# ffs97/deep-mixture-vae

Measured on AMD Instinct MI355X. Metric: images/sec (train), MNIST K=10 z=64 batch=4096/GPU bf16, higher is better.
Workload: dtype bf16; 1 GPU; configs[1]: DMVAE MLP 784-500-500-(2000|2000)-z64/K10-2000-500-500-784, one ELBO training step (gather+fwd+loss+bwd+Adam), synthetic rows resident in HBM; per_gpu_batch=4096, global_batch=4096, parallelism=dp1, rccl_ranks=0, multi_rank_rccl_verified_before_this_run=False, hip_graph=True, float_atomics=False, update=adam fused into the dW launch, mode=exact (expectation over q(c|x), priors.py:130-145)

## Files before the change

### deep-mixture-vae_amd/build.py

```python
import os
import subprocess
import sys
from concurrent.futures import ThreadPoolExecutor

HERE = os.path.dirname(os.path.abspath(__file__))
CSRC = os.path.join(HERE, "csrc")
OUT = os.path.join(HERE, "dmvae_hip", "libdmvae_hip.so")
SOURCES = ["gemm_bf16.hip", "gemm_bf16_256.hip", "gemm_f32.hip", "latent.hip", "latent_mfma.hip", "latent_vade.hip", "latent_vade_mfma.hip", "elementwise.hip", "conv.hip", "heads_dx.hip", "heads_latent.hip", "strip_fwd2.hip", "moe_head.hip", "gmm_fit.hip", "gmm_seed.hip", "eval_clusters.hip", "api.hip"]
FLAGS = ["--offload-arch=gfx950", "-O3", "-fPIC", "-std=c++17", "-Wall", "-Wno-unused-function",
         "-mllvm", "-amdgpu-mfma-vgpr-form=1"]


def _stale(target, deps):
    if not os.path.exists(target):
        return True
    t = os.path.getmtime(target)
    return any(os.path.getmtime(d) > t for d in deps)


def build(force=False, verbose=True):
    hipcc = os.environ.get("HIPCC", "/opt/rocm/bin/hipcc")
    headers = [os.path.join(CSRC, f) for f in os.listdir(CSRC) if f.endswith(".h")]
    headers += [os.path.join(HERE, "..", "include", h) for h in ("dmvae_hip.h", "dmvae_hip_debug.h")]
    objdir = os.path.join(HERE, "build")
    os.makedirs(objdir, exist_ok=True)
    os.makedirs(os.path.dirname(OUT), exist_ok=True)
    jobs = []
    objs = []
    for src in SOURCES:
        sp = os.path.join(CSRC, src)
        op = os.path.join(objdir, src.replace(".hip", ".o"))
        objs.append(op)
        if force or _stale(op, [sp] + headers):
            jobs.append([hipcc] + FLAGS + ["-c", sp, "-o", op])

    def run(cmd):
        if verbose:
            print(" ".join(cmd), flush=True)
        r = subprocess.run(cmd, capture_output=True, text=True)
        if r.returncode != 0:
            raise RuntimeError("hipcc failed:\n%s\n%s" % (" ".join(cmd), r.stderr[-6000:]))
        if verbose and r.stderr.strip():
            print(r.stderr[-3000:], file=sys.stderr)

    with ThreadPoolExecutor(max_workers=min(4, max(1, len(jobs)))) as ex:
        list(ex.map(run, jobs))
    if jobs or force or _stale(OUT, objs):
        run([hipcc, "--offload-arch=gfx950", "-shared", "-fPIC", "-o", OUT] + objs)
    return OUT


def build_host_asan(verbose=False):
    import glob
    hipcc = os.environ.get("HIPCC", "/opt/rocm/bin/hipcc")
    objdir = os.path.join(HERE, "build", "asan")
    os.makedirs(objdir, exist_ok=True)
    out = os.path.join(objdir, "libdmvae_hip_asan.so")
    headers = [os.path.join(CSRC, f) for f in os.listdir(CSRC) if f.endswith(".h")] + [os.path.join(HERE, "..", "include", h) for h in ("dmvae_hip.h", "dmvae_hip_debug.h")]
    flags = ["--offload-arch=gfx950", "--cuda-host-only", "-O1", "-g", "-fPIC", "-std=c++17", "-fsanitize=address,undefined", "-fno-gpu-sanitize",
             "-fno-omit-frame-pointer", "-fno-sanitize-recover=undefined"]
    objs, jobs = [], []
    for src in SOURCES:
        sp, op = os.path.join(CSRC, src), os.path.join(objdir, src.replace(".hip", ".o"))
        objs.append(op)
        if _stale(op, [sp] + headers):
            jobs.append([hipcc] + flags + ["-c", sp, "-o", op])

    def run(cmd):
        if verbose:
            print(" ".join(cmd), flush=True)
        r = subprocess.run(cmd, capture_output=True, text=True)
        if r.returncode != 0:
            raise RuntimeError("hipcc (host asan) failed:\n%s\n%s" % (" ".join(cmd), r.stderr[-6000:]))
    with ThreadPoolExecutor(max_workers=min(4, max(1, len(jobs)))) as ex:
        list(ex.map(run, jobs))
    if jobs or _stale(out, objs):
        und = subprocess.run(["nm", "-u"] + objs, capture_output=True, text=True).stdout
        syms = sorted({w for line in und.splitlines() for w in line.split() if w.startswith("__hip_fatbin_")})
        stub = os.path.join(objdir, "fatbin_stubs.c")
        with open(stub, "w") as f:
            for sname in syms:
                f.write('const char %s[32] __attribute__((aligned(4096))) = "__CLANG_OFFLOAD_BUNDLE__";\n' % sname)
        run(["gcc", "-c", "-fPIC", stub, "-o", stub.replace(".c", ".o")])
        run([hipcc, "--offload-arch=gfx950", "--cuda-host-only", "-shared", "-fPIC", "-fsanitize=address,undefined", "-fno-gpu-sanitize", "-shared-libsan", "-o", out]
            + objs + [stub.replace(".c", ".o")])
    rt = sorted(glob.glob("/opt/rocm/lib/llvm/lib/clang/*/lib/linux/libclang_rt.asan-x86_64.so"))
    return out, (rt[-1] if rt else None)


if __name__ == "__main__":
    print(build(force="-f" in sys.argv))
```

### deep-mixture-vae_amd/csrc/api.hip

```cpp
#include <stdarg.h>
#include <stdlib.h>
#include <string.h>

#include <map>
#include <mutex>
#include <string>
#include <vector>

#include "kernels.h"
#include "moe_head.h"
#include "gmm_fit.h"
#include "gmm_seed.h"
#include "eval_clusters.h"
#include "measure.h"

namespace dmvae {

static thread_local char g_err[512] = "";
void set_error(const char* fmt, ...) {
    va_list ap;
    va_start(ap, fmt);
    vsnprintf(g_err, sizeof(g_err), fmt, ap);
    va_end(ap);
}
// ... 1376 lines not shown
    DMVAE_REQUIRE(out && n > 0, "dmvae_philox_uniform: bad argument");
    return philox_launch((hipStream_t)stream, out, n, seed, step, sid, 2);
}
extern "C" int dmvae_philox_gumbel(void* stream, float* out, int64_t n, uint64_t seed, uint64_t step, uint32_t sid) {
    DMVAE_REQUIRE(out && n > 0, "dmvae_philox_gumbel: bad argument");
    return philox_launch((hipStream_t)stream, out, n, seed, step, sid, 1);
}
extern "C" int dmvae_cast_f32_to_bf16(void* stream, const float* in, void* out, int64_t n) {
    DMVAE_REQUIRE(in && out && n > 0, "dmvae_cast: bad argument");
    return cast_launch((hipStream_t)stream, in, out, n, 1);
}
extern "C" int dmvae_cast_bf16_to_f32(void* stream, const void* in, float* out, int64_t n) {
    DMVAE_REQUIRE(in && out && n > 0, "dmvae_cast: bad argument");
    return cast_launch((hipStream_t)stream, in, out, n, 0);
}

extern "C" int dmvae_debug_spin(void* stream, int microseconds) { return spin_launch((hipStream_t)stream, microseconds); }
extern "C" int dmvae_debug_strip_fwd2(void* stream, int B_pad, int K0, const void* X, int64_t ldx, const void* W0, int64_t ld0, const float* b0,
                                      const void* W1, int64_t ld1, const float* b1, void* Y1, int64_t ldy1, void* Y2, int64_t ldy2) {
    return strip_fwd2_launch((hipStream_t)stream, B_pad, K0, X, ldx, W0, ld0, b0, W1, ld1, b1, Y1, ldy1, Y2, ldy2);
}
extern "C" int dmvae_debug_stamps(void** device_ptr) {
    if (!device_ptr) return DMVAE_EINVAL;
    *device_ptr = gemm_bf16_stamps();
    if (!*device_ptr) *device_ptr = heads_dx_phase_table();
    return *device_ptr ? 0 : DMVAE_ESTATE;
}

extern "C" int dmvae_debug_anatomy(void** device_ptr) {
    if (!device_ptr) return DMVAE_EINVAL;
    *device_ptr = gemm_bf16_anatomy();
    return *device_ptr ? 0 : DMVAE_ESTATE;
}
extern "C" int dmvae_debug_anatomy256(void** device_ptr) {
    if (!device_ptr) return DMVAE_EINVAL;
    *device_ptr = gemm_bf16_256_anatomy();
    return *device_ptr ? 0 : DMVAE_ESTATE;
}

extern "C" int dmvae_debug_conv_first_fwd(void* stream, int dtype, const void* x, int64_t bstride, int H, int64_t n_img, const void* W, int ldw,
                                          const float* bias, void* out, int ld) {
    DMVAE_REQUIRE((dtype == DMVAE_F32 || dtype == DMVAE_BF16) && x && W && bias && out && H > 0 && n_img > 0 && bstride >= (int64_t)H * H, "dmvae_debug_conv_first_fwd: bad argument");
    return conv_first_fwd_launch((hipStream_t)stream, dtype, x, bstride, H, n_img, W, ldw, bias, 32, out, ld);
}
extern "C" int dmvae_debug_conv_first_dw(void* stream, int dtype, const void* x, int64_t bstride, int H, int64_t n_img, const void* dY, int ld,
                                         float* dW, int ldw, float* db, float* part, int64_t part_floats, int* n_blocks) {
    DMVAE_REQUIRE((dtype == DMVAE_F32 || dtype == DMVAE_BF16) && H > 0 && H % 4 == 0 && n_img > 0 && (ld == 32 || ld == 64) && n_blocks &&
                  n_img * H * (H / 4) < (1ll << 31), "dmvae_debug_conv_first_dw: bad argument (side a multiple of 4, ld 32 or 64)");
    *n_blocks = conv_first_dw_blocks(H, n_img);
    if (!part) return 0;
    DMVAE_REQUIRE(x && dY && dW && db && bstride >= (int64_t)H * H && part_floats >= (int64_t)*n_blocks * 320,
                  "dmvae_debug_conv_first_dw: bad argument (scratch: %d blocks x 320 floats)", *n_blocks);
    return conv_first_dw_launch((hipStream_t)stream, dtype, x, bstride, H, n_img, dY, ld, 32, dW, ldw, db, part);
}
extern "C" int dmvae_debug_zero_border(void* stream, int dtype, void* a, int P, int ld, int64_t n_img) {
    DMVAE_REQUIRE((dtype == DMVAE_F32 || dtype == DMVAE_BF16) && a && P >= 2 && n_img > 0, "dmvae_debug_zero_border: bad argument");
    return zero_border_launch((hipStream_t)stream, dtype, a, P, ld, n_img);
}
extern "C" int dmvae_debug_maxpool2_fwd(void* stream, int dtype, const void* in, int H, int ld, int64_t n_img, void* out, int out_border) {
    DMVAE_REQUIRE((dtype == DMVAE_F32 || dtype == DMVAE_BF16) && in && out && H > 0 && n_img > 0 && (out_border == 0 || out_border == 1), "dmvae_debug_maxpool2_fwd: bad argument");
    return maxpool2_fwd_launch((hipStream_t)stream, dtype, in, H, ld, n_img, out, out_border);
}
extern "C" int dmvae_debug_maxpool2_bwd_relu(void* stream, int dtype, const void* in, const void* dout, int H, int ld, int64_t n_img, void* din, int dout_border) {
    DMVAE_REQUIRE((dtype == DMVAE_F32 || dtype == DMVAE_BF16) && in && dout && din && H > 0 && n_img > 0 && (dout_border == 0 || dout_border == 1), "dmvae_debug_maxpool2_bwd_relu: bad argument");
    return maxpool2_bwd_relu_launch((hipStream_t)stream, dtype, in, dout, H, ld, n_img, din, dout_border);
}
extern "C" int dmvae_debug_conv_wflip(void* stream, int dtype, const void* W, int cin, int cin_ld, int cout, int ldw, void* Wt, int Kt) {
    DMVAE_REQUIRE((dtype == DMVAE_F32 || dtype == DMVAE_BF16) && W && Wt && cin > 0 && cout > 0 && ldw >= cout, "dmvae_debug_conv_wflip: bad argument");
    return conv_wflip_launch((hipStream_t)stream, dtype, W, cin, cin_ld, cout, ldw, Wt, Kt);
}
extern "C" int dmvae_debug_conv_gemm(void* stream, int dtype, int layout, int M, int N, int K, const void* A, int64_t lda,
                                     const void* B, int64_t ldb, const dmvae_epilogue* epi, int split_k, int conv_p, int conv_c) {
    DMVAE_REQUIRE(conv_p >= 3 && conv_c > 0, "dmvae_debug_conv_gemm: conv_p = side + 2 >= 3, conv_c > 0");
    return gemm_checked((hipStream_t)stream, dtype, layout, M, N, K, A, lda, B, ldb, epi, split_k, nullptr, conv_p, conv_c);
}
extern "C" int dmvae_debug_conv_dw(void* stream, int dtype, int rows, int conv_p, int conv_c, const void* X, int64_t ldx, const void* dY, int64_t ldy,
                                   int N, int n_valid, int split, float* slab, float* dW, float* db) {
    DMVAE_REQUIRE(rows > 0 && conv_p >= 3 && conv_c > 0 && N > 0 && n_valid > 0 && n_valid <= N && dW && db && split >= 1 && rows % (split * 64) == 0 && (split == 1 || slab),
                  "dmvae_debug_conv_dw: bad argument");
    const int kdim = pad64(9 * conv_c);
    hipError_t me = hipMemsetAsync(dW, 0, (size_t)kdim * N * 4, (hipStream_t)stream);
    if (me == hipSuccess) me = hipMemsetAsync(db, 0, (size_t)N * 4, (hipStream_t)stream);
    if (me != hipSuccess) { set_error("dmvae_debug_conv_dw memset: %s", hipGetErrorString(me)); return (int)me; }
    return conv_layer_dw((hipStream_t)stream, dtype, rows, conv_p, conv_c, kdim, X, ldx, dY, ldy, N, n_valid, split, slab, dW, db);
}

extern "C" int dmvae_prof_enable(int on) {
    std::lock_guard<std::mutex> lk(g_prof_mu);
    g_prof_on = on != 0;
    return 0;
}
extern "C" int dmvae_prof_collect(dmvae_prof_row* rows, int max_rows) {
    std::lock_guard<std::mutex> lk(g_prof_mu);
    std::map<std::string, dmvae_prof_row> agg;
    std::vector<std::string> order;
    for (auto& r : g_prof) {
        (void)hipEventSynchronize(r.e1);
        float ms = 0.f;
        (void)hipEventElapsedTime(&ms, r.e0, r.e1);
        double kms = 0.0;
        bool kok = !r.k.empty();
        for (auto& pr : r.k) {
            float d = 0.f;
            if (hipEventSynchronize(pr.second) != hipSuccess || hipEventElapsedTime(&d, pr.first, pr.second) != hipSuccess || !(d > 0.f)) kok = false;
            kms += d;
            g_event_pool.push_back(pr.first);
            g_event_pool.push_back(pr.second);
        }
        (void)hipGetLastError();
        auto it = agg.find(r.name);
        if (it == agg.end()) {
            dmvae_prof_row row;
            memset(&row, 0, sizeof(row));
            snprintf(row.name, sizeof(row.name), "%s", r.name);
            it = agg.emplace(r.name, row).first;
            order.push_back(r.name);
        }
        it->second.launches += 1;
        it->second.total_ms += ms;
        it->second.kernel_ms += kok ? kms : 0.0;
        it->second.kernel_launches += kok ? (int64_t)r.k.size() : 0;
        it->second.flops += r.flops;
        it->second.bytes += r.bytes;
        g_event_pool.push_back(r.e0);
        g_event_pool.push_back(r.e1);
    }
    g_prof.clear();
    g_prof_cur = -1;
    int n = 0;
    for (auto& k : order) {
        if (n >= max_rows) break;
        rows[n++] = agg[k];
    }
    return n;
}

extern "C" int dmvae_debug_set_tile(int bm, int bn) {
    DMVAE_REQUIRE((bm == 0 && bn == 0) || ((bm == 64 || bm == 128) && (bn == 64 || bn == 128)), "dmvae_debug_set_tile: 64 or 128 (0,0 = heuristic)");
    gemm_bf16_force_tile(bm * 1000 + bn);
    return 0;
}

extern "C" int dmvae_debug_set_knob(int which, int value) {
    if (which == 10) { g_dw_slices = value; return 0; }
    if (which == 11) { g_dw_macro = value; return 0; }
    if (which == 12) { g_heads_dx_form = value; return 0; }
    if (which == 13) { heads_dx_stream_set(value); return 0; }
    if (which == 16) { g_fin_rides = value; return 0; }
    if (which == 17) { g_pf_rides = value; return 0; }
    if (which == 18 || which == 20) { gemm_bf16_set_knob(which, value); return 0; }
    if (which == 19) { heads_latent_set(value); return 0; }
    if (which == 21) { g_ksplit = value; return 0; }
    if (which == 22) { latent_vade_force_mfma(value); return 0; }
    if (which == 14) { latent_set_blocks_target(value); return 0; }
    DMVAE_REQUIRE(which >= 0 && which <= 9 && which != 3, "dmvae_debug_set_knob: knob 0 = supertile rows, 1 = 8-wave workgroups, 2 = per-problem tiles in grouped grids, (3: removed, the deep-ring policy), 4 = XCD runs per tile class in grouped grids, 5 = short-K conv tiles, 6 = 256x256 tile policy, 7 = short-K workgroups, 8 = first-tile stagger of the merged dW grid, 9 = waves per workgroup of a grouped dX launch; 10 / 11 = K slices of the dW groups, 12 = heads dX as one or two launches, 13 = heads dX on the streaming kernel (1) or the grouped tiles (0), 14 = blocks the latent kernel's geometry aims at (512), 19 = fused heads + latent launch, 20 = XCD partition of the grouped dW launch, 21 = K slices of a small batch's thin launches, 22 = VaDE's large-table latent form wherever the caller brings its scratch");
    gemm_bf16_set_knob(which, value);
    return 0;
}

extern "C" int dmvae_abi_version(void) { return DMVAE_ABI_VERSION; }
extern "C" const char* dmvae_last_error(void) { return g_err; }
```

### deep-mixture-vae_amd/csrc/gemm_bf16.hip

```cpp
#include <algorithm>
#include <cmath>
#include <functional>
#include <map>
#include <mutex>
#include <string>
#include <vector>

#include "gemm_tile.h"
#include "measure.h"

MEAS_TABLES_BF16

namespace dmvae {

template <int BM, int BN, int LAYOUT, int EPI, int NSTAGE, int NW, int BKT = BK, bool CONV = false, bool BONLY = false>
__device__ __forceinline__ void gemm_bf16_body(const GemmArgs& a, const int bid_raw, const int gstart, const int nwg, bf16_t* smem,
                                               const dmvae_adam_ctx* ac = nullptr, const int kslice = -1) {
    constexpr bool A_KC = (LAYOUT != DMVAE_GEMM_DW);
    constexpr bool B_KC = (LAYOUT == DMVAE_GEMM_DX);
    constexpr int A_ELEMS = BM * BKT, B_ELEMS = BN * BKT, STAGE = A_ELEMS + B_ELEMS;
    constexpr int WM = NW / 2;
    constexpr int TM = BM / (16 * WM), TN = BN / 32;
    static_assert(!BONLY || (LAYOUT == DMVAE_GEMM_DW && EPI == DMVAE_EPI_STORE_F32 && !CONV), "bias-only strips: dense DW / STORE_F32");
    constexpr int LOADS = ((BONLY ? 0 : BM) + BN) * BKT / (512 * NW);
// ... 756 lines not shown
    return check_launch("gemm_bf16_grouped");
}

int gemm_bf16_grouped(hipStream_t s, int layout, const GemmArgs* probs, int nprob, const dmvae_finalize_args* fin) {
    if (nprob < 1 || nprob > DMVAE_MAX_GROUP) { set_error("dmvae_gemm_grouped: 1..%d problems", DMVAE_MAX_GROUP); return DMVAE_EINVAL; }
    const int epi = probs[0].epi.kind;
    for (int i = 1; i < nprob; ++i)
        if (probs[i].epi.kind != epi) { set_error("dmvae_gemm_grouped: all problems must share the epilogue kind"); return DMVAE_EINVAL; }
    if (layout == DMVAE_GEMM_DW && epi == DMVAE_EPI_STORE_F32) return grouped_launch<DMVAE_GEMM_DW, DMVAE_EPI_STORE_F32>(s, probs, nprob);
    if (layout == DMVAE_GEMM_FWD && epi == DMVAE_EPI_BIAS_F32) return grouped_launch<DMVAE_GEMM_FWD, DMVAE_EPI_BIAS_F32>(s, probs, nprob);
    if (fin && !(layout == DMVAE_GEMM_DX && epi == DMVAE_EPI_RELU_MASK)) { set_error("dmvae_gemm_grouped: step_finalize rides on DX / RELU_MASK groups only"); return DMVAE_EINVAL; }
    if (layout == DMVAE_GEMM_DX && epi == DMVAE_EPI_RELU_MASK) {
        bool taken[DMVAE_MAX_GROUP];
        const int rc = heads_dx_stream_launch(s, probs, nprob, fin, taken);
        if (rc) return rc;
        GemmArgs rest[DMVAE_MAX_GROUP];
        int nrest = 0, ntaken = 0;
        for (int i = 0; i < nprob; ++i) {
            if (taken[i]) ++ntaken;
            else rest[nrest++] = probs[i];
        }
        if (nrest == 0) return 0;
        return grouped_launch<DMVAE_GEMM_DX, DMVAE_EPI_RELU_MASK>(s, rest, nrest, nullptr, ntaken ? nullptr : fin);
    }
    set_error("dmvae_gemm_grouped: layout %d with epilogue %d is not instantiated", layout, epi);
    return DMVAE_EUNSUPPORTED;
}
static int peel_large_dw(hipStream_t s, const GemmArgs* probs, int nprob, const dmvae_adam_ctx* ctx, std::vector<GemmArgs>& rest) {
    std::vector<GemmArgs> large;
    bool any = false;
    for (int i = 0; i < nprob; ++i)
        any = any || (probs[i].k_split == probs[i].K && gemm_bf16_256_ok(DMVAE_GEMM_DW, probs[i].epi.kind, probs[i].M, probs[i].N, probs[i].K, probs[i].conv_c != 0));
    for (int i = 0; i < nprob; ++i) {
        const GemmArgs& p = probs[i];
        if (p.k_split != p.K && !p.bias_only && !p.epi.out2 && p.slab_stride && gemm_bf16_256_slice_ok(p.M, p.N, p.k_split)) { large.push_back(p); continue; }
        const bool own = p.k_split == p.K && gemm_bf16_256_ok(DMVAE_GEMM_DW, p.epi.kind, p.M, p.N, p.K, p.conv_c != 0);
        const bool rides = any && gemm_bf16_256_rides() && p.k_split == p.K && !p.conv_c && p.M % 256 == 0 && p.N % 256 == 0 && p.K >= 1024 &&
                           (p.epi.kind == DMVAE_EPI_STORE_F32 || p.epi.kind == DMVAE_EPI_ADAM);
        if (own || rides) large.push_back(p);
        else rest.push_back(p);
    }
    return large.empty() ? 0 : gemm_bf16_256_dw_all(s, large.data(), (int)large.size(), ctx);
}
int gemm_bf16_grouped_dw(hipStream_t s, const GemmArgs* probs, int nprob) {
    if (nprob < 1 || nprob > DMVAE_MAX_GROUP) { set_error("dmvae_gemm_grouped_dw: 1..%d problems", DMVAE_MAX_GROUP); return DMVAE_EINVAL; }
    std::vector<GemmArgs> rest;
    for (int i = 0; i < nprob; ++i)
        if (probs[i].epi.kind != DMVAE_EPI_STORE_F32) return gemm_bf16_grouped(s, DMVAE_GEMM_DW, probs, nprob, nullptr);
    const int rc = peel_large_dw(s, probs, nprob, nullptr, rest);
    if (rc) return rc;
    return rest.empty() ? 0 : gemm_bf16_grouped(s, DMVAE_GEMM_DW, rest.data(), (int)rest.size(), nullptr);
}
int gemm_bf16_grouped_dw_adam(hipStream_t s, const GemmArgs* probs, int nprob, const dmvae_adam_ctx& ctx) {
    if (nprob < 1 || nprob > DMVAE_MAX_GROUP) { set_error("dmvae_gemm_grouped_dw_adam: 1..%d problems", DMVAE_MAX_GROUP); return DMVAE_EINVAL; }
    for (int i = 0; i < nprob; ++i)
        if (probs[i].epi.kind != DMVAE_EPI_ADAM || !probs[i].epi.out) { set_error("dmvae_gemm_grouped_dw_adam: every problem needs epilogue kind ADAM and out = its gradient address"); return DMVAE_EINVAL; }
    if (!ctx.param || !ctx.grad || !ctx.m || !ctx.v || !ctx.state || (ctx.seg_off & 3) || (ctx.seg_n & 3) || ctx.seg_n < 0) {
        set_error("dmvae_gemm_grouped_dw_adam: null arena / state, or a segment that is not a multiple of 4 elements");
        return DMVAE_EINVAL;
    }
    for (int i = 0; i < nprob; ++i) {
        const int64_t end = (reinterpret_cast<const float*>(probs[i].epi.out) - ctx.grad) + (int64_t)probs[i].M * probs[i].epi.ldo;
        if (end < 0 || end > ADAM_QUADS_MAX_ELEMS) { set_error("dmvae_gemm_grouped_dw_adam: gradient %d ends %lld elements into the arena (limit 2^30)", i, (long long)end); return DMVAE_EUNSUPPORTED; }
    }
    std::vector<GemmArgs> rest;
    dmvae_adam_ctx c1 = ctx;
    c1.seg_n = 0;
    const int rc = peel_large_dw(s, probs, nprob, &c1, rest);
    if (rc) return rc;
    if (!rest.empty()) return grouped_launch<DMVAE_GEMM_DW, DMVAE_EPI_ADAM>(s, rest.data(), (int)rest.size(), &ctx);
    if (ctx.seg_n > 0) {
        AdamArgs a;
        a.n = ctx.seg_n; a.p = ctx.param + ctx.seg_off; a.g = ctx.grad + ctx.seg_off; a.m = ctx.m + ctx.seg_off; a.v = ctx.v + ctx.seg_off;
        a.pb = ctx.param_bf16 ? reinterpret_cast<bf16_t*>(ctx.param_bf16) + ctx.seg_off : nullptr;
        a.lr = 0.f; a.b1 = ctx.beta1; a.b2 = ctx.beta2; a.eps = ctx.epsilon; a.gscale = ctx.grad_scale; a.zero_grad = 0; a.ieee = ctx.ieee;
        a.t_host = ~0ull; a.st = reinterpret_cast<const dmvae_state*>(ctx.state);
        return adam_launch(s, a);
    }
    return 0;
}

static int g_force_tile = 0;
void gemm_bf16_force_tile(int t) { g_force_tile = t; }
static int g_nw8 = 1;
void gemm_bf16_set_knob(int which, int v) {
    if (which == 0) g_group_m = v < 0 ? 0 : v;
    if (which == 1) g_nw8 = v;
    if (which == 2) g_grouped_mixed = v;
    if (which == 4) g_grouped_cls = v;
    if (which == 5) g_conv_short = v;
    if (which == 6) gemm_bf16_256_set_policy(v);
    if (which == 7) g_shortk = v;
    if (which == 8) gemm_bf16_256_set_stagger(v);
    if (which == 9) g_dx_group_nw = v;
    if (which == 18) g_thin = v;
    if (which == 20) g_grouped_xcut = v;
}

static int gemm_bf16_thin_rows(const GemmArgs& a) {
    if (!g_thin || a.conv_c || a.N != 64 || a.K < 1024 || (a.k_split != a.K && !a.tick)) return 0;
    if (g_thin >= 2 && a.M % 16 == 0 && a.M / 16 <= 256) return 16;
    if (a.M % 32 == 0 && a.M / 32 <= 256) return 32;
    return 0;
}

int gemm_bf16_tile_m(int M, int N, int split) {
    if (g_force_tile) {
        const int bm = g_force_tile / 1000, bn = g_force_tile % 1000;
        if (M % bm == 0 && N % bn == 0) return g_force_tile;
    }
    static const int cand[4][2] = {{128, 128}, {128, 64}, {64, 128}, {64, 64}};
    double best = -1.0;
    int pick = 64 * 1000 + 64;
    for (auto& c : cand) {
        if (M % c[0] || N % c[1]) continue;
        const double wgs = (double)(M / c[0]) * (N / c[1]) * split;
        const double score = (double)c[0] * c[1] / (c[0] + c[1]) * (wgs >= 256.0 ? 1.0 : wgs / 256.0);
        if (score > best * 1.0001) { best = score; pick = c[0] * 1000 + c[1]; }
    }
    if (pick == 128128 && (double)(M / 128) * (N / 128) * split <= 256.0 && (double)(M / 128) * (N / 64) * split >= 384.0) pick = 128064;
    return pick;
}

template <int LAYOUT, int EPI>
static int launch_tiled(hipStream_t s, const GemmArgs& a0, int split, const GemmRiders* riders = nullptr) {
    GemmArgs a = a0;
    int t = gemm_bf16_tile_m(a.M, a.N, split);
    if (a.conv_c) {
        constexpr bool ok = (LAYOUT == DMVAE_GEMM_FWD && EPI == DMVAE_EPI_BIAS_RELU) || (LAYOUT == DMVAE_GEMM_DX && EPI == DMVAE_EPI_RELU_MASK) ||
                            (LAYOUT == DMVAE_GEMM_DW && (EPI == DMVAE_EPI_ATOMIC_F32 || EPI == DMVAE_EPI_STORE_F32));
        if constexpr (ok) {
            if (LAYOUT == DMVAE_GEMM_DW) t = 64 * 1000 + (a.N % 128 == 0 ? 128 : 64);
            a.group_m = gemm_auto_group_m(a.M / (t / 1000), a.N / (t % 1000), t / 1000, t % 1000);
            if constexpr (LAYOUT == DMVAE_GEMM_DW) {
                if (t == 64128) return launch_conv<64, 128, LAYOUT, EPI, 3>(s, a, split);
                if (g_conv_short == 2) return launch_conv<64, 64, LAYOUT, EPI, 3>(s, a, split);
                return launch_conv<64, 64, LAYOUT, EPI, 4>(s, a, split);
            } else {
                switch (t) {
                    case 128128: return launch_conv<128, 128, LAYOUT, EPI, 2, 8>(s, a, split);
                    case 128064:
                        if (a.K <= 640 && g_conv_short) return launch_conv<128, 64, LAYOUT, EPI, 2, 4>(s, a, split);
                        return launch_conv<128, 64, LAYOUT, EPI, 3, 8>(s, a, split);
                    case 64128: return launch_conv<64, 128, LAYOUT, EPI, 3>(s, a, split);
                    default: return launch_conv<64, 64, LAYOUT, EPI, 4>(s, a, split);
                }
            }
        } else {
            set_error("dmvae_gemm(bf16): conv mode is built for FWD+BIAS_RELU, DX+RELU_MASK and DW+ATOMIC_F32");
            return DMVAE_EUNSUPPORTED;
        }
    }
    if (riders && (a.conv_c || LAYOUT != DMVAE_GEMM_DX || gemm_bf16_256_ok(LAYOUT, EPI, a.M, a.N, a.K, false))) { set_error("gemm_bf16: riders are carried by the dense small-tile DX launches only (ask gemm_bf16_riders_room first)"); return DMVAE_EINVAL; }
    if (split == 1 && gemm_bf16_256_ok(LAYOUT, EPI, a.M, a.N, a.K, false)) return gemm_bf16_256_launch(s, LAYOUT, a);
    a.group_m = gemm_auto_group_m(a.M / (t / 1000), a.N / (t % 1000), t / 1000, t % 1000);
    if (g_shortk && a.K <= 128 && split == 1 && LAYOUT != DMVAE_GEMM_DW && EPI != DMVAE_EPI_BIAS_RECON) {
        a.group_m = gemm_auto_group_m(a.M / 64, a.N / 64, 64, 64);
        return launch<64, 64, LAYOUT, EPI, 2>(s, a, split, riders);
    }
    if constexpr (LAYOUT == DMVAE_GEMM_DX && EPI == DMVAE_EPI_LATENT) {
        const int thin = gemm_bf16_thin_rows(a);
        if (thin == 32) {
            a.group_m = gemm_auto_group_m(a.M / 32, a.N / 64, 32, 64);
            return launch<32, 64, LAYOUT, EPI, 4>(s, a, split, riders);
        }
        if (thin == 16) {
            if (riders && riders->nfin) { set_error("gemm_bf16: the 16-row tile (two waves) cannot carry the step_finalize blocks"); return DMVAE_EINVAL; }
            a.group_m = gemm_auto_group_m(a.M / 16, a.N / 64, 16, 64);
            return launch<16, 64, LAYOUT, EPI, 4, 2>(s, a, split, riders);
        }
    }
    switch (t) {
        case 128128:
            return g_nw8 ? launch<128, 128, LAYOUT, EPI, 2, 8>(s, a, split, riders) : launch<128, 128, LAYOUT, EPI, 2>(s, a, split, riders);
        case 128064:
            return g_nw8 ? launch<128, 64, LAYOUT, EPI, 3, 8>(s, a, split, riders) : launch<128, 64, LAYOUT, EPI, 3>(s, a, split, riders);
        case 64128: return launch<64, 128, LAYOUT, EPI, 3>(s, a, split, riders);
        default: return launch<64, 64, LAYOUT, EPI, 4>(s, a, split, riders);
    }
}

int gemm_bf16_riders_room(const GemmArgs& a, bool own_cu) {
    if (a.conv_c || gemm_bf16_256_ok(DMVAE_GEMM_DX, a.epi.kind, a.M, a.N, a.K, false)) return -1;
    if (a.epi.kind != DMVAE_EPI_LATENT && a.epi.kind != DMVAE_EPI_RELU_MASK) return -1;
    int t = gemm_bf16_tile_m(a.M, a.N, 1);
    if (g_shortk && a.K <= 128) t = 64064;
    if (a.epi.kind == DMVAE_EPI_LATENT && gemm_bf16_thin_rows(a)) t = gemm_bf16_thin_rows(a) * 1000 + 64;
    const int tiles = (a.M / (t / 1000)) * (a.N / (t % 1000));
    return (own_cu ? 256 : 512) - tiles;
}

bool gemm_bf16_carries_finalize(const GemmArgs& a) { return !(a.epi.kind == DMVAE_EPI_LATENT && gemm_bf16_thin_rows(a) == 16); }

int gemm_bf16_dispatch(hipStream_t s, int layout, const GemmArgs& a, int split, const GemmRiders* riders) {
    const int epi = a.epi.kind;
#define CASE(L, E) \
    if (layout == L && epi == E) return launch_tiled<L, E>(s, a, split, riders);
    CASE(DMVAE_GEMM_FWD, DMVAE_EPI_BIAS_RELU)
    CASE(DMVAE_GEMM_FWD, DMVAE_EPI_BIAS_F32)
    CASE(DMVAE_GEMM_FWD, DMVAE_EPI_BIAS_RECON)
    CASE(DMVAE_GEMM_FWD, DMVAE_EPI_BIAS_SIGMOID)
    CASE(DMVAE_GEMM_FWD, DMVAE_EPI_STORE_F32)
    CASE(DMVAE_GEMM_DX, DMVAE_EPI_STORE_F32)
    CASE(DMVAE_GEMM_DX, DMVAE_EPI_RELU_MASK)
    CASE(DMVAE_GEMM_DX, DMVAE_EPI_LATENT)
    CASE(DMVAE_GEMM_DW, DMVAE_EPI_STORE_F32)
    CASE(DMVAE_GEMM_DW, DMVAE_EPI_ATOMIC_F32)
#undef CASE
    set_error("dmvae_gemm(bf16): layout %d with epilogue %d is not instantiated", layout, epi);
    return DMVAE_EUNSUPPORTED;
}

}
```

### deep-mixture-vae_amd/csrc/kernels.h

```cpp
#pragma once
#include "gemm_epilogue.h"

namespace dmvae {

struct AdamArgs {
    int64_t n;
    float* p; float* g; float* m; float* v; bf16_t* pb;
    float lr, b1, b2, eps, gscale;
    int zero_grad;
    int ieee;
    uint64_t t_host;
    const dmvae_state* st;
};

#define DMVAE_MAX_GROUP 16
int gemm_bf16_dispatch(hipStream_t s, int layout, const GemmArgs& a, int split, const GemmRiders* riders = nullptr);
int gemm_bf16_riders_room(const GemmArgs& a, bool own_cu);
bool gemm_bf16_carries_finalize(const GemmArgs& a);
int gemm_bf16_grouped_dw(hipStream_t s, const GemmArgs* probs, int nprob);
int gemm_bf16_grouped(hipStream_t s, int layout, const GemmArgs* probs, int nprob, const dmvae_finalize_args* fin = nullptr);
dmvae_finalize_args step_finalize_args(const float* rp, int nr, const float* lp, int nl, float inv_B, void* st, int bump_adam,
                                       float b1, float b2, const float* part, int nblk, int ncol, float* gout);
int gemm_bf16_tile_m(int M, int N, int split);
int gemm_auto_group_m(int tiles_m, int tiles_n, int bm, int bn, double run = 0.0);
bool gemm_bf16_256_ok(int layout, int epi, int M, int N, int K, bool conv);
int gemm_bf16_256_launch(hipStream_t s, int layout, const GemmArgs& a, const dmvae_adam_ctx* ctx = nullptr);
void gemm_bf16_256_set_policy(int v);
void gemm_bf16_256_set_stagger(int v);
bool gemm_bf16_256_slice_ok(int M, int N, int k_split);
bool gemm_bf16_256_rides();
int gemm_bf16_256_dw_all(hipStream_t s, const GemmArgs* probs, int n, const dmvae_adam_ctx* ctx);
void* heads_dx_phase_table();
int heads_dx_stream_launch(hipStream_t s, const GemmArgs* probs, int nprob, const dmvae_finalize_args* fin, bool* taken);
void heads_dx_stream_set(int v);
void gemm_bf16_force_tile(int t);
void gemm_bf16_set_knob(int which, int v);
int gemm_f32_dispatch(hipStream_t s, int layout, const GemmArgs& a, int split);
int gemm_f32_trio(hipStream_t s, const GemmArgs& g1, int split1, const GemmArgs& g2, int split2, const GemmArgs& g3, int split3);
int latent_nblocks(int B_pad, int D, int K);
int latent_launch(hipStream_t s, const dmvae_latent_args* a);
void latent_set_blocks_target(int v);
int latent_vade_nblocks(int B_pad);
int latent_vade_launch(hipStream_t s, const dmvae_latent_args* a);
size_t latent_vade_lds_bytes(int D, int K);
bool latent_vade_mfma_needed(int D, int K);
bool latent_vade_mfma_forced();
void latent_vade_force_mfma(int v);
int64_t latent_vade_mfma_ws_bytes(int B_pad, int D, int K, int* n_slabs);
int latent_vade_mfma_launch(hipStream_t s, const dmvae_latent_args* a, float* ws, int64_t ws_bytes);
bool heads_latent_ok(int B_pad, int D, int K, int Dp, int Kp, int Hp, int mode, int rows_per_latent_block);
int heads_latent_launch(hipStream_t s, const dmvae_latent_args* a, const dmvae_heads_args* h);
void heads_latent_set(int v);
int64_t heads_latent_kslice_floats(int B_pad, int Dp, int slices);
int strip_fwd2_launch(hipStream_t s, int B_pad, int K0, const void* X, int64_t ldx, const void* W0, int64_t ld0, const float* b0,
                      const void* W1, int64_t ld1, const float* b1, void* Y1, int64_t ldy1, void* Y2, int64_t ldy2);
bool latent_mfma_applies(int D, int K, int mode);
int64_t latent_mfma_ws_bytes(int B_pad, int D, int K);
int latent_mfma_launch(hipStream_t s, const dmvae_latent_args* a, float* ws, int64_t ws_bytes);
int adam_launch(hipStream_t s, const AdamArgs& a);
int adam_shadow_launch(hipStream_t s, const AdamArgs& a, int blocks);
int adam_finish_launch(hipStream_t s, void* st);
int adam_slabs_launch(hipStream_t s, const AdamArgs& a, const float* slabs, int nslab, int64_t stride, int64_t seg_lo, int64_t seg_hi);
int slab_reduce_launch(hipStream_t s, const float* slabs, int64_t n, int nslab, int64_t stride, float* out);
int colsum_prepare(int64_t max_n);
float* colsum_global_scratch(int64_t* elems);
int colsum_launch(hipStream_t s, int in_dtype, const void* in, int64_t ld, int M, int N, float* out, float* ws, int64_t ws_elems);
int recon_nblocks(int B_pad, int I_pad);
int recon_launch(hipStream_t s, int act_dtype, int recon_kind, int B, int B_pad, int I, int I_pad, const float* logits, int64_t ldl,
                 const float* x, int64_t ldx, float inv_B, void* dl, int64_t ldd, float* partials);
int loss_finalize_launch(hipStream_t s, const float* rp, int nr, const float* lp, int nl, float inv_B, void* st, int bump_adam);
int step_finalize_launch(hipStream_t s, const float* rp, int nr, const float* lp, int nl, float inv_B, void* st, int bump_adam,
                         float b1, float b2, const float* part, int nblk, int ncol, float* gout);
int gemm_bf16_grouped_dw_adam(hipStream_t s, const GemmArgs* probs, int nprob, const dmvae_adam_ctx& ctx);
dmvae_gather_args gather_args(int act_dtype, const float* data, int64_t n_rows, int dim, const int32_t* perm, int64_t first, int batch, int n_valid,
                              int B_pad, void* out_act, int64_t ld_act, float* out_f32, int64_t ld_f32, int cols_pad, const void* st);
int gather_launch(hipStream_t s, int act_dtype, const float* data, int64_t n_rows, int dim, const int32_t* perm, int64_t first, int batch,
                  int n_valid, int B_pad, void* out_act, int64_t ld_act, float* out_f32, int64_t ld_f32, int cols_pad, const void* st);
int philox_launch(hipStream_t s, float* out, int64_t n, uint64_t seed, uint64_t step, uint32_t sid, int gumbel);
int cast_launch(hipStream_t s, const void* in, void* out, int64_t n, int to_bf16);
int spin_launch(hipStream_t s, int us);
void* gemm_bf16_stamps();
void* gemm_bf16_anatomy();
void* gemm_bf16_256_anatomy();
int conv_first_fwd_launch(hipStream_t s, int dtype, const void* x, int64_t bstride, int H, int64_t n_img, const void* W, int ldw,
                          const float* bias, int cout, void* out, int ld);
int conv_first_dw_blocks(int H, int64_t n_img);
int conv_first_dw_launch(hipStream_t s, int dtype, const void* x, int64_t bstride, int H, int64_t n_img, const void* dY, int ld, int cout,
                         float* dW, int ldw, float* db, float* part);
int zero_border_launch(hipStream_t s, int dtype, void* a, int P, int ld, int64_t n_img);
int maxpool2_fwd_launch(hipStream_t s, int dtype, const void* in, int H, int ld, int64_t n_img, void* out, int out_border);
int maxpool2_bwd_relu_launch(hipStream_t s, int dtype, const void* in, const void* dout, int H, int ld, int64_t n_img, void* din, int dout_border);
int conv_wflip_launch(hipStream_t s, int dtype, const void* W, int cin, int cin_ld, int cout, int ldw, void* Wt, int Kt);

}
```

Before: 15.06 million images/sec.

## Add weight-stationary streaming GEMM for K=512 forward and dX layers

Adds a new kernel for K=512 GEMMs with a bias+ReLU epilogue (forward) or a ReLU-mask epilogue (dX). Each workgroup keeps a 128-column weight slice resident in registers and streams 64-row A tiles through double-buffered LDS, prefetching the next tile and its gates while computing the current one. The goal is to avoid reloading weights for every output tile and to overlap loads with MFMA work on the tall-skinny layers, such as 4096x2000x512. It is on by default for M>=4096 and N>=2048. Because N must be a multiple of 128, shapes like N=500 keep the old path.

```diff
diff --git a/deep-mixture-vae_amd/build.py b/deep-mixture-vae_amd/build.py
--- a/deep-mixture-vae_amd/build.py
+++ b/deep-mixture-vae_amd/build.py
@@ -6,7 +6,7 @@
 HERE = os.path.dirname(os.path.abspath(__file__))
 CSRC = os.path.join(HERE, "csrc")
 OUT = os.path.join(HERE, "dmvae_hip", "libdmvae_hip.so")
-SOURCES = ["gemm_bf16.hip", "gemm_bf16_256.hip", "gemm_f32.hip", "latent.hip", "latent_mfma.hip", "latent_vade.hip", "latent_vade_mfma.hip", "elementwise.hip", "conv.hip", "heads_dx.hip", "heads_latent.hip", "strip_fwd2.hip", "moe_head.hip", "gmm_fit.hip", "gmm_seed.hip", "eval_clusters.hip", "api.hip"]
+SOURCES = ["gemm_bf16.hip", "gemm_bf16_256.hip", "gemm_f32.hip", "latent.hip", "latent_mfma.hip", "latent_vade.hip", "latent_vade_mfma.hip", "elementwise.hip", "conv.hip", "heads_dx.hip", "gemm_stream.hip", "heads_latent.hip", "strip_fwd2.hip", "moe_head.hip", "gmm_fit.hip", "gmm_seed.hip", "eval_clusters.hip", "api.hip"]
 FLAGS = ["--offload-arch=gfx950", "-O3", "-fPIC", "-std=c++17", "-Wall", "-Wno-unused-function",
          "-mllvm", "-amdgpu-mfma-vgpr-form=1"]
 
diff --git a/deep-mixture-vae_amd/csrc/api.hip b/deep-mixture-vae_amd/csrc/api.hip
--- a/deep-mixture-vae_amd/csrc/api.hip
+++ b/deep-mixture-vae_amd/csrc/api.hip
@@ -1552,8 +1552,9 @@
     if (which == 19) { heads_latent_set(value); return 0; }
     if (which == 21) { g_ksplit = value; return 0; }
     if (which == 22) { latent_vade_force_mfma(value); return 0; }
+    if (which == 23) { gemm_stream_set(value); return 0; }
     if (which == 14) { latent_set_blocks_target(value); return 0; }
-    DMVAE_REQUIRE(which >= 0 && which <= 9 && which != 3, "dmvae_debug_set_knob: knob 0 = supertile rows, 1 = 8-wave workgroups, 2 = per-problem tiles in grouped grids, (3: removed, the deep-ring policy), 4 = XCD runs per tile class in grouped grids, 5 = short-K conv tiles, 6 = 256x256 tile policy, 7 = short-K workgroups, 8 = first-tile stagger of the merged dW grid, 9 = waves per workgroup of a grouped dX launch; 10 / 11 = K slices of the dW groups, 12 = heads dX as one or two launches, 13 = heads dX on the streaming kernel (1) or the grouped tiles (0), 14 = blocks the latent kernel's geometry aims at (512), 19 = fused heads + latent launch, 20 = XCD partition of the grouped dW launch, 21 = K slices of a small batch's thin launches, 22 = VaDE's large-table latent form wherever the caller brings its scratch");
+    DMVAE_REQUIRE(which >= 0 && which <= 9 && which != 3, "dmvae_debug_set_knob: knob 0 = supertile rows, 1 = 8-wave workgroups, 2 = per-problem tiles in grouped grids, (3: removed, the deep-ring policy), 4 = XCD runs per tile class in grouped grids, 5 = short-K conv tiles, 6 = 256x256 tile policy, 7 = short-K workgroups, 8 = first-tile stagger of the merged dW grid, 9 = waves per workgroup of a grouped dX launch; 10 / 11 = K slices of the dW groups, 12 = heads dX as one or two launches, 13 = heads dX on the streaming kernel (1) or the grouped tiles (0), 14 = blocks the latent kernel's geometry aims at (512), 19 = fused heads + latent launch, 20 = XCD partition of the grouped dW launch, 21 = K slices of a small batch's thin launches, 22 = VaDE's large-table latent form wherever the caller brings its scratch, 23 = streaming GEMM of the K = 512 layers (0 never, 1 the rule, 2 every admissible shape)");
     gemm_bf16_set_knob(which, value);
     return 0;
 }
diff --git a/deep-mixture-vae_amd/csrc/gemm_bf16.hip b/deep-mixture-vae_amd/csrc/gemm_bf16.hip
--- a/deep-mixture-vae_amd/csrc/gemm_bf16.hip
+++ b/deep-mixture-vae_amd/csrc/gemm_bf16.hip
@@ -932,6 +932,10 @@
         }
     }
     if (riders && (a.conv_c || LAYOUT != DMVAE_GEMM_DX || gemm_bf16_256_ok(LAYOUT, EPI, a.M, a.N, a.K, false))) { set_error("gemm_bf16: riders are carried by the dense small-tile DX launches only (ask gemm_bf16_riders_room first)"); return DMVAE_EINVAL; }
+    if (split == 1 && !riders && !g_force_tile && gemm_stream_ok(LAYOUT, EPI, a.M, a.N, a.K)) {
+        const int rc = gemm_stream_launch(s, LAYOUT, a);
+        if (rc >= 0) return rc;
+    }
     if (split == 1 && gemm_bf16_256_ok(LAYOUT, EPI, a.M, a.N, a.K, false)) return gemm_bf16_256_launch(s, LAYOUT, a);
     a.group_m = gemm_auto_group_m(a.M / (t / 1000), a.N / (t % 1000), t / 1000, t % 1000);
     if (g_shortk && a.K <= 128 && split == 1 && LAYOUT != DMVAE_GEMM_DW && EPI != DMVAE_EPI_BIAS_RECON) {
diff --git a/deep-mixture-vae_amd/csrc/gemm_stream.hip b/deep-mixture-vae_amd/csrc/gemm_stream.hip
--- /dev/null
+++ b/deep-mixture-vae_amd/csrc/gemm_stream.hip
@@ -0,0 +1,258 @@
+#include <algorithm>
+#include <string>
+#include <type_traits>
+
+#include "gemm_tile.h"
+
+namespace dmvae {
+namespace {
+
+typedef unsigned u32x2 __attribute__((ext_vector_type(2)));
+
+__device__ __forceinline__ void gld2(u32x2& d, const void* p) { asm volatile("global_load_dwordx2 %0, %1, off" : "=v"(d) : "v"(p) : "memory"); }
+__device__ __forceinline__ void gst2(void* p, u32x2 d) { asm volatile("global_store_dwordx2 %0, %1, off\n\ts_nop 1" ::"v"(p), "v"(d) : "memory"); }
+template <int N>
+__device__ __forceinline__ void wait_gates(u32x2 (&g)[4]) {
+    asm volatile("s_waitcnt vmcnt(%4)" : "+v"(g[0]), "+v"(g[1]), "+v"(g[2]), "+v"(g[3]) : "n"(N) : "memory");
+}
+__device__ __forceinline__ void lds_done() { asm volatile("s_waitcnt lgkmcnt(0)" ::: "memory"); }
+
+#ifndef DMVAE_STREAM_ABLATE
+#define DMVAE_STREAM_ABLATE 0
+#endif
+constexpr int ABL = DMVAE_STREAM_ABLATE;
+constexpr int CW = 128;
+constexpr int NW = 8;
+constexpr int NT = 64 * NW;
+constexpr int SLOTS = 256;
+constexpr int MIN_STEPS = 4;
+
+template <int LAYOUT, int KS>
+__device__ __forceinline__ void gemm_stream_body(const GemmArgs& a, const int slice, const int t0, const int steps, bf16_t* smem) {
+    constexpr bool DXL = LAYOUT == DMVAE_GEMM_DX;
+    constexpr int K = 32 * KS, KT = K / 64, CB = 2;
+    constexpr int SLOT = KT * 4096;
+    constexpr int NQ = 64 * (CW / 4) / NT;
+    constexpr int NAG = KT;
+    static_assert(KS % 2 == 0 && NQ == 4 && CW == 16 * CB * (NW / 2) && 2 * NQ + NAG <= 63, "tile shape / vmcnt range");
+    const int tid = threadIdx.x, lane = tid & 63;
+    const int wave = __builtin_amdgcn_readfirstlane(tid >> 6);
+    const int wm = wave >> 2, wn = wave & 3, li = lane & 15, g = lane >> 4;
+    const int n0 = slice * CW;
+    bf16_t* As = smem;
+    float* ct = reinterpret_cast<float*>(smem + 2 * SLOT);
+    const unsigned lds_a = __builtin_amdgcn_readfirstlane((unsigned)(size_t)((__attribute__((address_space(3))) bf16_t*)As) + 1024u * (unsigned)wave);
+
+    const bf16_t* Ag = reinterpret_cast<const bf16_t*>(a.A) + (int64_t)t0 * 64 * a.lda;
+    const bf16_t* Wg = reinterpret_cast<const bf16_t*>(a.B) + (DXL ? (int64_t)n0 * a.ldb : (int64_t)n0);
+    const int64_t stepW = DXL ? (int64_t)64 : (int64_t)64 * a.ldb;
+    unsigned goA[1], goW[2];
+    stage_offsets<64, true, NW, 64>(a.lda, wave, lane, goA);
+    stage_offsets<CW, DXL, NW, 64>(a.ldb, wave, lane, goW);
+
+    auto issue_a = [&](int s) {
+        const bf16_t* src = Ag + (int64_t)s * 64 * a.lda;
+        const unsigned dst = lds_a + 2u * (unsigned)((s & 1) * SLOT);
+#pragma unroll
+        for (int kt = 0; kt < KT; ++kt) glds_tile(src + kt * 64, goA, dst + 2u * (unsigned)(kt * 4096), 0u);
+    };
+    constexpr int RQ = NT / (CW / 4);
+    const int ml0 = tid / (CW / 4), cq = tid % (CW / 4);
+    float* cq_p = ct + ml0 * CW + ((cq ^ (ml0 & 7)) << 2);
+    const bf16_t* gate_p = DXL ? reinterpret_cast<const bf16_t*>(a.epi.aux0) + (int64_t)(t0 * 64 + ml0) * a.epi.ld0 + n0 + cq * 4 : nullptr;
+    bf16_t* out_p = reinterpret_cast<bf16_t*>(a.epi.out) + (int64_t)(t0 * 64 + ml0) * a.epi.ldo + n0 + cq * 4;
+    auto issue_gates = [&](u32x2 (&gt)[NQ], int s) {
+#pragma unroll
+        for (int q = 0; q < NQ; ++q) gld2(gt[q], gate_p + ((int64_t)s * 64 + q * RQ) * a.epi.ld0);
+    };
+    auto park_gates = [&](const u32x2 (&gt)[NQ]) {
+#pragma unroll
+        for (int q = 0; q < NQ; ++q) *reinterpret_cast<u32x2*>(cq_p + q * RQ * CW) = gt[q];
+    };
+
+    float bq[4] = {0.f, 0.f, 0.f, 0.f};
+    if constexpr (!DXL) loadf4(a.epi.bias, n0 + cq * 4, bq);
+#pragma unroll
+    for (int kt = 0; kt < KT; ++kt) glds_tile(Wg + kt * stepW, goW, lds_a + 2u * (unsigned)(kt * CW * 64), 1024u * NW);
+    bf16x8 wf[CB][KS];
+    {
+        u32x2 g0[NQ];
+        if constexpr (DXL) {
+            issue_gates(g0, 0);
+            wait_gates<0>(g0);
+        } else {
+            wait_vmcnt<0>();
+            asm volatile("" : "+v"(bq[0]), "+v"(bq[1]), "+v"(bq[2]), "+v"(bq[3]));
+        }
+        __builtin_amdgcn_s_barrier();
+#pragma unroll
+        for (int j = 0; j < CB; ++j)
+#pragma unroll
+            for (int kk = 0; kk < KS; ++kk) {
+                unsigned short lo, hi;
+                frag_offsets<CW, DXL>(wn * 32 + j * 16, kk & 1, lane, lo, hi);
+                wf[j][kk] = read_frag<DXL>(As + (kk >> 1) * CW * 64, lo, hi);
+            }
+        lds_done();
+        __builtin_amdgcn_sched_barrier(0);
+        if constexpr (DXL) park_gates(g0);
+    }
+    unsigned short foA[2][2];
+#pragma unroll
+    for (int i = 0; i < 2; ++i)
+#pragma unroll
+        for (int ks = 0; ks < 2; ++ks) { unsigned short hi; frag_offsets<64, true>(wm * 32 + i * 16, ks, lane, foA[i][ks], hi); }
+    lds_done();
+    __builtin_amdgcn_s_barrier();
+    issue_a(0);
+
+    auto step = [&](auto firstc, auto lastc, int s) {
+        constexpr bool FIRST = decltype(firstc)::value, LAST = decltype(lastc)::value;
+        u32x2 gt[NQ];
+        if constexpr (DXL) {
+#pragma unroll
+            for (int q = 0; q < NQ; ++q) gt[q] = *reinterpret_cast<const u32x2*>(cq_p + q * RQ * CW);
+            lds_done();
+        }
+        if constexpr (FIRST) wait_vmcnt<0>();
+        __builtin_amdgcn_s_barrier();
+        u32x2 gn[NQ];
+        if constexpr (!LAST) {
+            if constexpr (DXL) issue_gates(gn, s + 1);
+            if constexpr (!(ABL & 4)) issue_a(s + 1);
+        }
+        const bf16_t* Ab = As + (s & 1) * SLOT;
+        bf16x8 af[2][2][2];
+        auto rd = [&](int kt) {
+#pragma unroll
+            for (int i = 0; i < 2; ++i)
+#pragma unroll
+                for (int ks = 0; ks < 2; ++ks) af[kt & 1][i][ks] = read_frag<true>(Ab + kt * 4096, foA[i][ks], 0);
+        };
+        f32x4 acc[2][CB];
+#pragma unroll
+        for (int i = 0; i < 2; ++i)
+#pragma unroll
+            for (int j = 0; j < CB; ++j) acc[i][j] = f32x4{0.f, 0.f, 0.f, 0.f};
+        rd(0);
+#pragma unroll
+        for (int kt = 0; kt < KT; ++kt) {
+            if (kt + 1 < KT && !(ABL & 8)) rd(kt + 1);
+            __builtin_amdgcn_s_setprio(1);
+#pragma unroll
+            for (int ks = 0; ks < 2; ++ks)
+#pragma unroll
+                for (int i = 0; i < 2; ++i)
+#pragma unroll
+                    for (int j = 0; j < CB; ++j) {
+                        if constexpr (ABL & 2) asm volatile("" ::"v"(wf[j][kt * 2 + ks]), "v"(af[kt & 1][i][ks]));
+                        else acc[i][j] = __builtin_amdgcn_mfma_f32_16x16x32_bf16(wf[j][kt * 2 + ks], af[kt & 1][i][ks], acc[i][j], 0, 0, 0);
+                    }
+            __builtin_amdgcn_s_setprio(0);
+        }
+#pragma unroll
+        for (int i = 0; i < 2; ++i)
+#pragma unroll
+            for (int j = 0; j < CB; ++j) {
+                const int ml = wm * 32 + i * 16 + li;
+                const int c = (wn * 32 + j * 16) / 4 + g;
+                *reinterpret_cast<f32x4*>(ct + ml * CW + ((c ^ (ml & 7)) << 2)) = acc[i][j];
+            }
+        lds_done();
+        __builtin_amdgcn_s_barrier();
+#pragma unroll
+        for (int q = 0; q < NQ; ++q) {
+            const f32x4 t = *reinterpret_cast<const f32x4*>(cq_p + q * RQ * CW);
+            float v0, v1, v2, v3;
+            if constexpr (DXL) {
+                v0 = __uint_as_float(gt[q][0] << 16) > 0.f ? t[0] : 0.f;
+                v1 = __uint_as_float(gt[q][0] & 0xffff0000u) > 0.f ? t[1] : 0.f;
+                v2 = __uint_as_float(gt[q][1] << 16) > 0.f ? t[2] : 0.f;
+                v3 = __uint_as_float(gt[q][1] & 0xffff0000u) > 0.f ? t[3] : 0.f;
+            } else {
+                v0 = fmaxf(t[0] + bq[0], 0.f);
+                v1 = fmaxf(t[1] + bq[1], 0.f);
+                v2 = fmaxf(t[2] + bq[2], 0.f);
+                v3 = fmaxf(t[3] + bq[3], 0.f);
+            }
+            u32x2 o;
+            o[0] = pack2bf(v0, v1);
+            o[1] = pack2bf(v2, v3);
+            if constexpr (ABL & 1) asm volatile("" ::"v"(o));
+            else gst2(out_p + ((int64_t)s * 64 + q * RQ) * a.epi.ldo, o);
+        }
+        constexpr int NST = (ABL & 1) ? 0 : NQ;
+        if constexpr (!LAST) {
+            if constexpr (DXL) {
+                wait_gates<NST>(gn);
+                park_gates(gn);
+            } else {
+                wait_vmcnt<NST>();
+            }
+        }
+    };
+    using T = std::true_type; using F = std::false_type;
+    if (steps == 1) { step(T{}, T{}, 0); return; }
+    step(T{}, F{}, 0);
+    int s = 1;
+    for (; s + 1 < steps; ++s) step(F{}, F{}, s);
+    step(F{}, T{}, s);
+}
+
+}
+
+struct StreamGrid { int nsl, chunks, steps; };
+
+template <int LAYOUT, int KS>
+__global__ __launch_bounds__(NT, 1) void gemm_stream_kernel(GemmArgs a, StreamGrid gr) {
+    __shared__ __attribute__((aligned(16))) bf16_t smem[2 * (KS / 2) * 4096 + 64 * CW * 2];
+    const int bx = (int)blockIdx.x;
+    const int chunk = bx / gr.nsl, slice = bx - chunk * gr.nsl;
+    const int tiles = a.M / 64;
+    const int t0 = chunk * gr.steps;
+    const int steps = min(gr.steps, tiles - t0);
+    if (chunk >= gr.chunks || steps <= 0) return;
+    gemm_stream_body<LAYOUT, KS>(a, slice, t0, steps, smem);
+}
+
+static int g_gemm_stream = 1;
+void gemm_stream_set(int v) { g_gemm_stream = v; }
+
+bool gemm_stream_ok(int layout, int epi, int M, int N, int K) {
+    if (g_gemm_stream == 0) return false;
+    const bool pair = (layout == DMVAE_GEMM_FWD && epi == DMVAE_EPI_BIAS_RELU) || (layout == DMVAE_GEMM_DX && epi == DMVAE_EPI_RELU_MASK);
+    if (!pair || K != 512 || M <= 0 || N <= 0 || M % 64 || N % CW || N / CW > SLOTS) return false;
+    if (g_gemm_stream >= 2) return true;
+    return M >= 4096 && N >= 2048;
+}
+
+static bool gemm_stream_aligned(int layout, const GemmArgs& p) {
+    if (p.conv_c || p.k_split != p.K || p.tick || p.bias_only || !p.A || !p.B || !p.epi.out) return false;
+    if ((p.lda * 2) % 16 || (p.ldb * 2) % 16 || p.epi.ldo % 8) return false;
+    if (((uintptr_t)p.epi.out | (uintptr_t)p.A | (uintptr_t)p.B) % 16) return false;
+    if (layout == DMVAE_GEMM_DX) return p.epi.aux0 && p.epi.ld0 % 8 == 0 && (uintptr_t)p.epi.aux0 % 16 == 0;
+    return p.epi.bias && (uintptr_t)p.epi.bias % 16 == 0;
+}
+
+int gemm_stream_launch(hipStream_t s, int layout, const GemmArgs& a) {
+    if (!gemm_stream_ok(layout, a.epi.kind, a.M, a.N, a.K) || !gemm_stream_aligned(layout, a)) return -1;
+    StreamGrid gr;
+    const int tiles = a.M / 64;
+    gr.nsl = a.N / CW;
+    gr.chunks = std::max(1, std::min(tiles, SLOTS / gr.nsl));
+    gr.steps = (tiles + gr.chunks - 1) / gr.chunks;
+    gr.steps = std::max(gr.steps, std::min(tiles, MIN_STEPS));
+    gr.chunks = (tiles + gr.steps - 1) / gr.steps;
+    const double flops = 2.0 * a.M * a.N * (double)a.K;
+    const double bytes = 2.0 * ((double)a.M * a.K + (double)a.K * a.N) + 2.0 * a.M * a.N + (layout == DMVAE_GEMM_DX ? 2.0 * a.M * a.N : 0.0);
+    if (layout == DMVAE_GEMM_DX) {
+        ProfScope ps(s, "gemm_stream_kernel<1, 16>", flops, bytes);
+        DMVAE_LAUNCH((gemm_stream_kernel<DMVAE_GEMM_DX, 16>), dim3(gr.chunks * gr.nsl), dim3(NT), 0, s, a, gr);
+    } else {
+        ProfScope ps(s, "gemm_stream_kernel<0, 16>", flops, bytes);
+        DMVAE_LAUNCH((gemm_stream_kernel<DMVAE_GEMM_FWD, 16>), dim3(gr.chunks * gr.nsl), dim3(NT), 0, s, a, gr);
+    }
+    return check_launch("gemm_stream");
+}
+
+}
diff --git a/deep-mixture-vae_amd/csrc/kernels.h b/deep-mixture-vae_amd/csrc/kernels.h
--- a/deep-mixture-vae_amd/csrc/kernels.h
+++ b/deep-mixture-vae_amd/csrc/kernels.h
@@ -33,6 +33,9 @@
 void* heads_dx_phase_table();
 int heads_dx_stream_launch(hipStream_t s, const GemmArgs* probs, int nprob, const dmvae_finalize_args* fin, bool* taken);
 void heads_dx_stream_set(int v);
+bool gemm_stream_ok(int layout, int epi, int M, int N, int K);
+int gemm_stream_launch(hipStream_t s, int layout, const GemmArgs& a);
+void gemm_stream_set(int v);
 void gemm_bf16_force_tile(int t);
 void gemm_bf16_set_knob(int which, int v);
 int gemm_f32_dispatch(hipStream_t s, int layout, const GemmArgs& a, int split);
```

Result: no change. 15.06 million images/sec (median of 3 runs) (+0.0%).
